# mosure/bevy_gaussian_splatting

Measured on NVIDIA H100. Metric: rendered Msplats/sec @1080p, 6M-gaussian cloud, higher is better.
Workload: dtype f32 (f16-packed inputs)

## Files before the change

bevy_gaussian_splatting_b200/csrc/raster.cu:

```cuda
#include <cuda_fp16.h>

#include "common.cuh"

namespace bgs {

constexpr int RT_THREADS = 256;
constexpr int RT_CHUNK = 256;

__device__ __forceinline__ void mbar_init(uint32_t bar, uint32_t count) {
    asm volatile("mbarrier.init.shared::cta.b64 [%0], %1;" ::"r"(bar), "r"(count) : "memory");
}
__device__ __forceinline__ void mbar_expect_tx(uint32_t bar, uint32_t bytes) {
    asm volatile("mbarrier.arrive.expect_tx.shared::cta.b64 _, [%0], %1;" ::"r"(bar), "r"(bytes) : "memory");
}
__device__ __forceinline__ void tma_bulk_g2s(uint32_t dst, const void* src, uint32_t bytes, uint32_t bar) {
    asm volatile("cp.async.bulk.shared::cluster.global.mbarrier::complete_tx::bytes [%0], [%1], %2, [%3];"
                 ::"r"(dst), "l"(src), "r"(bytes), "r"(bar) : "memory");
}
__device__ __forceinline__ void mbar_wait(uint32_t bar, uint32_t parity) {
    asm volatile(
        "{\n\t.reg .pred p;\n\t"
        "WAIT_%=:\n\t"
        "mbarrier.try_wait.parity.shared::cta.b64 p, [%0], %1;\n\t"
        "@p bra DONE_%=;\n\t"
        "bra WAIT_%=;\n\t"
        "DONE_%=:\n\t}" ::"r"(bar), "r"(parity) : "memory");
}
constexpr uint32_t ENT_WORDS = RT_CHUNK + 8;

struct PairStream {
    const uint32_t* entries;
    uint32_t (*ent)[ENT_WORDS];
    uint32_t a_ent, a_bar, end;
    bool tma;
    uint32_t issued = 0u, chunk = 0u;

    __device__ __forceinline__ PairStream(const uint32_t* tile_entries, uint32_t (*s_ent)[ENT_WORDS], unsigned long long* s_bar,
                                          uint2 range, bool use_tma)
        : entries(tile_entries), ent(s_ent), a_ent((uint32_t)__cvta_generic_to_shared(s_ent)),
          a_bar((uint32_t)__cvta_generic_to_shared(s_bar)), end(range.y), tma(use_tma) {
        if (!tma) return;
        if (threadIdx.x == 0) {
            mbar_init(a_bar, 1u); mbar_init(a_bar + 8u, 1u);
            asm volatile("fence.mbarrier_init.release.cluster;" ::: "memory");
        }
        __syncthreads();
        if (threadIdx.x == 0) issue(range.x, (uint32_t)RT_CHUNK, 0);
        issued = 1u;
    }
    __device__ __forceinline__ void issue(uint32_t base, uint32_t cnt, int buf) const {
        const uint32_t lead = base & 3u;
        const uint32_t bytes = ((lead + cnt) * 4u + 15u) & ~15u;
        mbar_expect_tx(a_bar + 8u * buf, bytes);
        tma_bulk_g2s(a_ent + (uint32_t)buf * ENT_WORDS * 4u, entries + (base - lead), bytes, a_bar + 8u * buf);
    }
    __device__ __forceinline__ void next(uint32_t base) {
        const int buf = (int)(chunk & 1u);
        if (tma) {
            if (base + RT_CHUNK < end) {
                if (threadIdx.x == 0) issue(base + RT_CHUNK, min((uint32_t)RT_CHUNK, end - base - RT_CHUNK), buf ^ 1);
                ++issued;
            }
            mbar_wait(a_bar + 8u * buf, (chunk >> 1) & 1u);
        }
    }
    template <class Index>
    __device__ __forceinline__ uint32_t entry(uint32_t base, Index j) const {
        return tma ? ent[chunk & 1u][(base & 3u) + j] : __ldg(entries + base + j);
    }
    __device__ __forceinline__ void finish() const {
        if (threadIdx.x == 0 && issued > chunk) mbar_wait(a_bar + 8u * (chunk & 1u), (chunk >> 1) & 1u);
    }
};

__device__ __forceinline__ void centre_out_tile(int b, int tiles_x, int tiles_y, int& tile_x, int& tile_y) {
    const int k = b / tiles_x, mid = tiles_y / 2;
    tile_x = b - k * tiles_x;
    tile_y = (k & 1) ? mid - (k + 1) / 2 : mid + k / 2;
}

__device__ __forceinline__ float linear_to_srgb(float c) {
    c = fminf(fmaxf(c, 0.0f), 1.0f);
    return c <= 0.0031308f ? 12.92f * c : 1.055f * __powf(c, 1.0f / 2.4f) - 0.055f;
}

constexpr uint32_t OUT_PREMUL = 1u, OUT_OVER = 2u;
__device__ __forceinline__ float srgb_decode(float c) {
    return c <= 0.04045f ? c * (1.0f / 12.92f) : __powf((c + 0.055f) * (1.0f / 1.055f), 2.4f);
}
__device__ __forceinline__ float4 read_pixel(const void* out, uint32_t fmt, size_t pix) {
    if (fmt == BGS_FORMAT_RGBA32F) return reinterpret_cast<const float4*>(out)[pix];
    if (fmt == BGS_FORMAT_RGBA16F) {
        const uint2 v = reinterpret_cast<const uint2*>(out)[pix];
        const float2 lo = __half22float2(*reinterpret_cast<const __half2*>(&v.x)), hi = __half22float2(*reinterpret_cast<const __half2*>(&v.y));
        return make_float4(lo.x, lo.y, hi.x, hi.y);
    }
    const uint32_t v = reinterpret_cast<const uint32_t*>(out)[pix];
    return make_float4(srgb_decode((float)(v & 255u) * (1.0f / 255.0f)), srgb_decode((float)((v >> 8) & 255u) * (1.0f / 255.0f)),
                       srgb_decode((float)((v >> 16) & 255u) * (1.0f / 255.0f)), (float)(v >> 24) * (1.0f / 255.0f));
}
__device__ __forceinline__ uint2 pack_rgba16f(float r, float g, float b, float a) {
    const __half2 lo = __floats2half2_rn(r, g), hi = __floats2half2_rn(b, a);
    return make_uint2(*reinterpret_cast<const uint32_t*>(&lo), *reinterpret_cast<const uint32_t*>(&hi));
}
__device__ __forceinline__ uint32_t pack_srgb8(float r, float g, float b, float a, bool with_alpha) {
    const uint32_t r8 = (uint32_t)(linear_to_srgb(r) * 255.0f + 0.5f);
    const uint32_t g8 = (uint32_t)(linear_to_srgb(g) * 255.0f + 0.5f);
    const uint32_t b8 = (uint32_t)(linear_to_srgb(b) * 255.0f + 0.5f);
    const uint32_t a8 = with_alpha ? (uint32_t)(fminf(fmaxf(a, 0.0f), 1.0f) * 255.0f + 0.5f) : 255u;
    return r8 | (g8 << 8) | (b8 << 16) | (a8 << 24);
}
__device__ __forceinline__ void write_pixel(void* out, uint32_t format, size_t pix, float r, float g, float b, float T) {
    const uint32_t fmt = format & 0xFFu, mode = format >> 8;
    float a = 1.0f;
    if (mode & OUT_OVER) {
        const float4 d = read_pixel(out, fmt, pix);
        r = fmaf(T, d.x, r); g = fmaf(T, d.y, g); b = fmaf(T, d.z, b);
        a = fmaf(T, d.w, 1.0f - T);
    } else if (mode & OUT_PREMUL) {
        a = 1.0f - T;
    }
    if (fmt == BGS_FORMAT_RGBA32F) {
        reinterpret_cast<float4*>(out)[pix] = make_float4(r, g, b, a);
    } else if (fmt == BGS_FORMAT_RGBA16F) {
        reinterpret_cast<uint2*>(out)[pix] = pack_rgba16f(r, g, b, a);
    } else {
        reinterpret_cast<uint32_t*>(out)[pix] = pack_srgb8(r, g, b, a, mode != 0);
    }
}

constexpr uint32_t SM_Q0 = 0;
constexpr uint32_t SM_UV = SM_Q0 + RT_CHUNK * 16;
constexpr uint32_t SM_Q2 = SM_UV + RT_CHUNK * 16;
constexpr uint32_t SM_LIST = SM_Q2 + RT_CHUNK * 16;
constexpr uint32_t SM_EXTRA = SM_LIST + (RT_THREADS / 32) * RT_CHUNK * 2;
constexpr uint32_t SM_BYTES = SM_EXTRA;
constexpr uint32_t SM_BYTES_2D = SM_EXTRA + 4 * RT_CHUNK * 16;

constexpr uint32_t REC_UV = SM_UV - SM_Q0, REC_Q2 = SM_Q2 - SM_Q0;
static_assert(REC_UV == RT_CHUNK * 16 && REC_Q2 == 2 * RT_CHUNK * 16, "q0, uv, q2 are consecutive float4 [RT_CHUNK] arrays");

__device__ __forceinline__ float4 lds4(uint32_t a) {
    float4 r; asm volatile("ld.shared.v4.f32 {%0,%1,%2,%3}, [%4];" : "=f"(r.x), "=f"(r.y), "=f"(r.z), "=f"(r.w) : "r"(a)); return r;
}
__device__ __forceinline__ float2 lds2(uint32_t a) {
    float2 r; asm volatile("ld.shared.v2.f32 {%0,%1}, [%2];" : "=f"(r.x), "=f"(r.y) : "r"(a)); return r;
}
__device__ __forceinline__ uint32_t lds_u16(uint32_t a) { uint32_t r; asm volatile("ld.shared.u16 %0, [%1];" : "=r"(r) : "r"(a)); return r; }
__device__ __forceinline__ uint32_t lds_u32(uint32_t a) { uint32_t r; asm volatile("ld.shared.u32 %0, [%1];" : "=r"(r) : "r"(a)); return r; }

__device__ __forceinline__ float2 quad_uv(float fx, float fy, float4 q0, float2 q1) {
    const float dx = __fsub_rn(fx, q0.x), dy = __fsub_rn(fy, q0.y);
    return make_float2(__fmaf_rn(q0.w, dy, __fmul_rn(q0.z, dx)), __fmaf_rn(q1.y, dy, __fmul_rn(q1.x, dx)));
}

template <class Hit>
__device__ __forceinline__ uint32_t compact_candidates(uint32_t cnt, unsigned short* list, uint32_t rec0, Hit hit) {
    uint32_t nl = 0;
    for (uint32_t j0 = 0; j0 < cnt; j0 += 32) {
        const uint32_t j = j0 + (threadIdx.x & 31u);
        bool h = false;
        if (j < cnt) h = hit(j);
        const uint32_t m = __ballot_sync(0xffffffffu, h);
        if (h) list[nl + __popc(m & lanemask_lt())] = (unsigned short)(rec0 + j * 16u);
        nl += __popc(m);
    }
    __syncwarp();
    return nl;
}

template <int MODE, bool AUX>
__global__ void __launch_bounds__(RT_THREADS, (MODE == 0 && !AUX) ? 6 : 5)
raster_kernel(const SplatRec* __restrict__ recs, const float4* __restrict__ extra, const uint32_t* __restrict__ tile_entries,
              const uint2* __restrict__ ranges, int W, int H, int tiles_x, void* __restrict__ out, uint32_t format,
              const float4* __restrict__ aux, void* __restrict__ out_depth, void* __restrict__ out_normal) {
    __shared__ __align__(16) unsigned char s_mem[(MODE == 2 ? SM_BYTES_2D : SM_BYTES) + (AUX ? 2 * RT_CHUNK * 16 : 0)];
    constexpr uint32_t SM_AUX = MODE == 2 ? SM_BYTES_2D : SM_BYTES;
    __shared__ __align__(16) uint32_t s_ent[2][ENT_WORDS];
    __shared__ __align__(8) unsigned long long s_bar[2];
    __shared__ __align__(8) float2 s_thr[MODE == 0 ? RT_CHUNK : 1];
    float4* s_q0 = reinterpret_cast<float4*>(s_mem + SM_Q0);
    float4* s_uv = reinterpret_cast<float4*>(s_mem + SM_UV);
    float4* s_q2 = reinterpret_cast<float4*>(s_mem + SM_Q2);
    const int t = threadIdx.x, lane = t & 31, warp = t >> 5;
    unsigned short* s_list = reinterpret_cast<unsigned short*>(s_mem + SM_LIST) + warp * RT_CHUNK;
    const uint32_t a_base = (uint32_t)__cvta_generic_to_shared(s_mem);
    const uint32_t a_list = a_base + SM_LIST + (uint32_t)warp * RT_CHUNK * 2u;
    int tile_x, tile_y;
    centre_out_tile((int)blockIdx.x, tiles_x, (int)gridDim.x / tiles_x, tile_x, tile_y);
    const int tile = tile_y * tiles_x + tile_x;
    const int wx0 = tile_x * TILE_PX + (warp & 1) * 8, wy0 = tile_y * TILE_PX + (warp >> 1) * 4;
    const int px = wx0 + (lane & 7), py = wy0 + (lane >> 3);
    const bool inside = px < W && py < H;
    const float fx = (float)px + 0.5f, fy = (float)py + 0.5f;
    const float rcx = (float)wx0 + 4.0f, rcy = (float)wy0 + 2.0f;
    const float tcx = (float)(tile_x * TILE_PX) + 8.0f, tcy = (float)(tile_y * TILE_PX) + 8.0f;
    uint2 range = ranges[tile];
    range.x = ~range.x;

    if (range.x >= range.y) {
        if (inside && !((format >> 8) & OUT_OVER)) {
            write_pixel(out, format, (size_t)py * W + px, 0.f, 0.f, 0.f, 1.0f);
            if (AUX) {
                write_pixel(out_depth, format, (size_t)py * W + px, 0.f, 0.f, 0.f, 1.0f);
                write_pixel(out_normal, format, (size_t)py * W + px, 0.f, 0.f, 0.f, 1.0f);
            }
        }
        return;
    }
    PairStream ps(tile_entries, s_ent, s_bar, range, range.y - range.x > (uint32_t)RT_CHUNK);

    float T = inside ? 1.0f : 0.0f, cr = 0.0f, cg = 0.0f, cb = 0.0f;
    float dr = 0.0f, dg = 0.0f, db = 0.0f, nr = 0.0f, ng = 0.0f, nb = 0.0f;
    for (uint32_t base = range.x; base < range.y; base += RT_CHUNK, ++ps.chunk) {
        if (__syncthreads_count(T < T_STOP ? 0 : 1) == 0) break;
        const uint32_t cnt = min((uint32_t)RT_CHUNK, range.y - base);
        ps.next(base);
        if ((uint32_t)t < cnt) {
            const uint32_t r = ps.entry(base, t);
            const float4* rp = reinterpret_cast<const float4*>(recs + r);
            const float4 p0 = __ldg(rp), p1 = __ldg(rp + 1);
            s_q0[t] = p0;
            s_uv[t] = p1;
            s_q2[t] = __ldg(rp + 2);
            if (MODE == 0) {
                const float ax = fabsf(p0.x - tcx) + 4.0f, ay = fabsf(p0.y - tcy) + 6.0f;
                const float ur = fabsf(p0.z) * 3.5f + fabsf(p0.w) * 1.5f, vr = fabsf(p1.x) * 3.5f + fabsf(p1.y) * 1.5f;
                const float um = fabsf(p0.z) * ax + fabsf(p0.w) * ay + ur, vm = fabsf(p1.x) * ax + fabsf(p1.y) * ay + vr;
                s_thr[t] = make_float2(ur + 1.0f + 1e-5f * um, vr + 1.0f + 1e-5f * vm);
            }
            if (MODE == 2) {
                float4* s_ex = reinterpret_cast<float4*>(s_mem + SM_EXTRA);
                const float4* ep = extra + (size_t)r * 4;
#pragma unroll
                for (int q = 0; q < 4; ++q) s_ex[q * RT_CHUNK + t] = __ldg(ep + q);
            }
            if (AUX) {
                float4* s_ax = reinterpret_cast<float4*>(s_mem + SM_AUX);
                s_ax[t] = __ldg(aux + (size_t)r * 2);
                s_ax[RT_CHUNK + t] = __ldg(aux + (size_t)r * 2 + 1);
            }
        }
        __syncthreads();
        const uint32_t nl = !__any_sync(0xffffffffu, !(T < T_STOP)) ? 0u : compact_candidates(cnt, s_list, a_base, [&](uint32_t j) {
            const float4 q = s_uv[j];
            const uint32_t bx = __float_as_uint(q.z), by = __float_as_uint(q.w);
            bool hit = !((int)(bx >> 16) < wx0 | (int)(bx & 0xFFFFu) > wx0 + 7 | (int)(by >> 16) < wy0 |
                         (int)(by & 0xFFFFu) > wy0 + 3);
            if (MODE == 0 && hit) {
                const float4 p = s_q0[j];
                const float2 th = s_thr[j];
                const float dxc = rcx - p.x, dyc = rcy - p.y;
                hit = !(fabsf(p.z * dxc + p.w * dyc) > th.x || fabsf(q.x * dxc + q.y * dyc) > th.y);
            }
            return hit;
        });
        if (MODE == 0 && !AUX) {
            const uint32_t a_end = a_list + nl * 2u;
            uint32_t a_it = a_list;
            float lim = (T < T_STOP) ? -1.0f : 1.0f;
            auto blend_if_covered = [&](uint32_t a_rec, float2 uv) {
                asm volatile(
                    "{\n\t"
                    ".reg .pred p, q;\n\t"
                    ".reg .f32 au, av, x, y, z, o, qd, e, a, w, na;\n\t"
                    "abs.f32 au, %5;\n\t"
                    "abs.f32 av, %6;\n\t"
                    "setp.le.f32 p, au, %4;\n\t"
                    "setp.le.and.f32 p, av, %4, p;\n\t"
                    "ld.shared.v4.f32 {x, y, z, o}, [%7+%8];\n\t"
                    "mul.rn.f32 qd, %5, %5;\n\t"
                    "fma.rn.f32 qd, %6, %6, qd;\n\t"
                    "mul.rn.f32 qd, qd, 0fC0CFBF83;\n\t"
                    "ex2.approx.ftz.f32 e, qd;\n\t"
                    "mul.rn.f32 a, e, o;\n\t"
                    "min.f32 a, a, 0f3F7FBE77;\n\t"
                    "mul.rn.f32 w, a, %0;\n\t"
                    "neg.f32 na, a;\n\t"
                    "@p fma.rn.f32 %1, w, x, %1;\n\t"
                    "@p fma.rn.f32 %2, w, y, %2;\n\t"
                    "@p fma.rn.f32 %3, w, z, %3;\n\t"
                    "@p fma.rn.f32 %0, na, %0, %0;\n\t"
                    "setp.lt.and.f32 q, %0, 0f38D1B717, p;\n\t"
                    "@q mov.f32 %4, 0fBF800000;\n\t"
                    "}"
                    : "+f"(T), "+f"(cr), "+f"(cg), "+f"(cb), "+f"(lim)
                    : "f"(uv.x), "f"(uv.y), "r"(a_rec), "n"(REC_Q2));
            };
            for (; a_it + 2u < a_end; a_it += 4u) {
                const uint32_t two = lds_u32(a_it);
                const uint32_t ra = two & 0xFFFFu, rb = two >> 16;
                const float4 pa = lds4(ra), pb = lds4(rb);
                const float2 sa = lds2(ra + REC_UV), sb = lds2(rb + REC_UV);
                const float2 uva = quad_uv(fx, fy, pa, sa), uvb = quad_uv(fx, fy, pb, sb);
                blend_if_covered(ra, uva);
                blend_if_covered(rb, uvb);
            }
            if (a_it != a_end) {
                const uint32_t ra = lds_u16(a_it);
                const float4 pa = lds4(ra);
                const float2 sa = lds2(ra + REC_UV);
                blend_if_covered(ra, quad_uv(fx, fy, pa, sa));
            }
        } else if (!(T < T_STOP)) {
            const uint32_t a_end = a_list + nl * 2u;
            for (uint32_t a_it = a_list; a_it != a_end; a_it += 2u) {
                const uint32_t a_rec = lds_u16(a_it);
                const float4 q0 = lds4(a_rec);
                const float2 q1 = lds2(a_rec + REC_UV);
                float e;
                float4 q2;
                if (MODE == 0) {
                    const float2 uv = quad_uv(fx, fy, q0, q1);
                    if (!(fabsf(uv.x) <= 1.0f && fabsf(uv.y) <= 1.0f)) continue;
                    const float qd = __fmaf_rn(uv.y, uv.y, __fmul_rn(uv.x, uv.x));
                    q2 = lds4(a_rec + REC_Q2);
                    asm("ex2.approx.ftz.f32 %0, %1;" : "=f"(e) : "f"(qd * -6.492127684f));
                } else {
                    const float dx = __fsub_rn(fx, q0.x), dy = __fsub_rn(fy, q0.y);
                    const float mx = __fadd_rn(dx, dx), my = -__fadd_rn(dy, dy);
                    const float Rq = q1.y;
                    float power;
                    if (MODE == 1) {
                        if (!(fabsf(mx) <= Rq && fabsf(my) <= Rq)) continue;
                        const float ddx = -mx, ddy = -my;
                        const float t1 = __fmul_rn(__fmul_rn(q0.z, ddx), ddx), t2 = __fmul_rn(__fmul_rn(q1.x, ddy), ddy);
                        power = __fadd_rn(__fmul_rn(-0.5f, __fadd_rn(t1, t2)), __fmul_rn(__fmul_rn(q0.w, ddx), ddy));
                    } else {
                        const float4 e0 = lds4(a_rec + SM_EXTRA);
                        if (!(fabsf(mx) <= e0.x && fabsf(my) <= e0.x)) continue;
                        const float4 e1 = lds4(a_rec + SM_EXTRA + RT_CHUNK * 16);
                        const float4 e2 = lds4(a_rec + SM_EXTRA + 2 * RT_CHUNK * 16);
                        const float4 e3 = lds4(a_rec + SM_EXTRA + 3 * RT_CHUNK * 16);
                        const float pcx = __fadd_rn(mx, e0.y), pcy = __fadd_rn(__fmul_rn(my, e0.w), e0.z);
                        const float hux = __fsub_rn(__fmul_rn(pcx, e3.x), e1.x), huy = __fsub_rn(__fmul_rn(pcx, e3.y), e1.y),
                                    huz = __fsub_rn(__fmul_rn(pcx, e3.z), e1.z);
                        const float hvx = __fsub_rn(__fmul_rn(pcy, e3.x), e2.x), hvy = __fsub_rn(__fmul_rn(pcy, e3.y), e2.y),
                                    hvz = __fsub_rn(__fmul_rn(pcy, e3.z), e2.z);
                        const float cpx = __fsub_rn(__fmul_rn(huy, hvz), __fmul_rn(huz, hvy));
                        const float cpy = __fsub_rn(__fmul_rn(huz, hvx), __fmul_rn(hux, hvz));
                        const float cpz = __fsub_rn(__fmul_rn(hux, hvy), __fmul_rn(huy, hvx));
                        const float us = __fdiv_rn(cpx, cpz), vs = __fdiv_rn(cpy, cpz);
                        const float s3 = __fadd_rn(__fmul_rn(us, us), __fmul_rn(vs, vs));
                        const float ex = __fsub_rn(e0.y, pcx), ey = __fsub_rn(e0.z, pcy);
                        const float s2 = __fmul_rn(2.0f, __fadd_rn(__fmul_rn(ex, ex), __fmul_rn(ey, ey)));
                        power = -__fmul_rn(0.5f, fminf(s3, s2));
                    }
                    if (power > 0.0f) continue;
                    q2 = lds4(a_rec + REC_Q2);
                    e = __expf(power);
                }
                const float a = fminf(e * q2.w, 0.999f);
                const float w = a * T;
                cr = fmaf(w, q2.x, cr); cg = fmaf(w, q2.y, cg); cb = fmaf(w, q2.z, cb);
                if (AUX) {
                    const float4 ad = lds4(a_rec + SM_AUX), an = lds4(a_rec + SM_AUX + RT_CHUNK * 16);
                    dr = fmaf(w, ad.x, dr); dg = fmaf(w, ad.y, dg); db = fmaf(w, ad.z, db);
                    nr = fmaf(w, an.x, nr); ng = fmaf(w, an.y, ng); nb = fmaf(w, an.z, nb);
                }
                T = fmaf(-a, T, T);
                if (T < T_STOP) break;
            }
        }
    }
    ps.finish();
    if (!inside) return;
    write_pixel(out, format, (size_t)py * W + px, cr, cg, cb, T);
    if (AUX) {
        write_pixel(out_depth, format, (size_t)py * W + px, dr, dg, db, T);
        write_pixel(out_normal, format, (size_t)py * W + px, nr, ng, nb, T);
    }
}

constexpr int R2_THREADS = 128;
constexpr uint32_t R2_LIST = SM_Q2 + RT_CHUNK * 16;
constexpr uint32_t R2_BYTES = R2_LIST + (R2_THREADS / 32) * RT_CHUNK * 2;

__device__ __forceinline__ void store_pixel2(void* out, uint32_t format, size_t pix, bool in0, bool in1, float r0, float g0,
                                             float b0, float r1, float g1, float b1, float T0, float T1) {
    if (format >> 8) {
        if (in0) write_pixel(out, format, pix, r0, g0, b0, T0);
        if (in1) write_pixel(out, format, pix + 1, r1, g1, b1, T1);
        return;
    }
    if (format == BGS_FORMAT_RGBA32F) {
        float4* o = reinterpret_cast<float4*>(out) + pix;
        if (in0) o[0] = make_float4(r0, g0, b0, 1.0f);
        if (in1) o[1] = make_float4(r1, g1, b1, 1.0f);
    } else if (format == BGS_FORMAT_RGBA16F) {
        uint2* o = reinterpret_cast<uint2*>(out) + pix;
        const uint2 p0 = pack_rgba16f(r0, g0, b0, 1.0f), p1 = pack_rgba16f(r1, g1, b1, 1.0f);
        if (in0) o[0] = p0;
        if (in1) o[1] = p1;
    } else {
        uint32_t* o = reinterpret_cast<uint32_t*>(out) + pix;
        const uint32_t p0 = pack_srgb8(r0, g0, b0, 1.0f, false), p1 = pack_srgb8(r1, g1, b1, 1.0f, false);
        if (in0 && in1 && (pix & 1) == 0) *reinterpret_cast<uint2*>(o) = make_uint2(p0, p1);
        else { if (in0) o[0] = p0; if (in1) o[1] = p1; }
    }
}

template <bool CHUNKED>
__global__ void __launch_bounds__(R2_THREADS)
raster2_kernel(const SplatRec* __restrict__ recs, const uint32_t* __restrict__ tile_entries, const uint2* __restrict__ ranges,
               int W, int H, int tiles_x, void* __restrict__ out, uint32_t format, float4* __restrict__ state,
               unsigned char* __restrict__ tile_done, uint32_t* __restrict__ tiles_done, int first, int last) {
    __shared__ __align__(16) unsigned char s_mem[R2_BYTES];
    float4* s_q0 = reinterpret_cast<float4*>(s_mem + SM_Q0);
    float4* s_uv = reinterpret_cast<float4*>(s_mem + SM_UV);
    float4* s_q2 = reinterpret_cast<float4*>(s_mem + SM_Q2);
    const int t = threadIdx.x, lane = t & 31, warp = t >> 5;
    unsigned short* s_list = reinterpret_cast<unsigned short*>(s_mem + R2_LIST) + warp * RT_CHUNK;
    const uint32_t a_base = (uint32_t)__cvta_generic_to_shared(s_mem);
    const uint32_t a_list = a_base + R2_LIST + (uint32_t)warp * RT_CHUNK * 2u;
    int tile_x, tile_y;
    centre_out_tile((int)blockIdx.x, tiles_x, (int)gridDim.x / tiles_x, tile_x, tile_y);
    const int tile = tile_y * tiles_x + tile_x;
    const int wy0 = tile_y * TILE_PX + warp * 4;
    const int px0 = tile_x * TILE_PX + 2 * (lane & 7), py = wy0 + (lane >> 3);
    const bool in0 = px0 < W && py < H, in1 = px0 + 1 < W && py < H;
    const float fx0 = (float)px0 + 0.5f, fx1 = (float)px0 + 1.5f, fy = (float)py + 0.5f;
    uint2 range = ranges[tile];
    range.x = ~range.x;

    float T0 = in0 ? 1.0f : 0.0f, T1 = in1 ? 1.0f : 0.0f;
    float lim0 = in0 ? 1.0f : -1.0f, lim1 = in1 ? 1.0f : -1.0f;
    float r0 = 0.f, g0 = 0.f, b0 = 0.f, r1 = 0.f, g1 = 0.f, b1 = 0.f;
    float4* st = nullptr;
    if (CHUNKED) {
        st = state + ((size_t)tile * R2_THREADS + t) * 2;
        if (!first) {
            const bool done = tile_done[tile] != 0;
            if (!last && (done || range.x >= range.y)) return;
            const float4 s0 = st[0], s1 = st[1];
            r0 = s0.x; g0 = s0.y; b0 = s0.z; T0 = s0.w;
            r1 = s1.x; g1 = s1.y; b1 = s1.z; T1 = s1.w;
            lim0 = (in0 && !(T0 < T_STOP)) ? 1.0f : -1.0f;
            lim1 = (in1 && !(T1 < T_STOP)) ? 1.0f : -1.0f;
            if (done) range.y = range.x;
        }
    }
    __shared__ __align__(16) uint32_t s_ent[2][ENT_WORDS];
    __shared__ __align__(8) unsigned long long s_bar[2];
    PairStream ps(tile_entries, s_ent, s_bar, range, range.y > range.x && range.y - range.x > (uint32_t)RT_CHUNK);
    for (uint32_t base = range.x; base < range.y; base += RT_CHUNK, ++ps.chunk) {
        if (__syncthreads_count((lim0 > 0.f || lim1 > 0.f) ? 1 : 0) == 0) break;
        const uint32_t cnt = min((uint32_t)RT_CHUNK, range.y - base);
        ps.next(base);
#pragma unroll
        for (int k = 0; k < RT_CHUNK / R2_THREADS; ++k) {
            const uint32_t j = t + k * R2_THREADS;
            if (j < cnt) {
                const uint32_t r = ps.entry(base, j);
                const float4* rp = reinterpret_cast<const float4*>(recs + r);
                s_q0[j] = __ldg(rp);
                s_uv[j] = __ldg(rp + 1);
                s_q2[j] = __ldg(rp + 2);
            }
        }
        __syncthreads();
        const uint32_t nl = !__any_sync(0xffffffffu, lim0 > 0.f || lim1 > 0.f) ? 0u : compact_candidates(cnt, s_list, 0u, [&](uint32_t j) {
            const uint32_t by = __float_as_uint(s_uv[j].w);
            return !((int)(by >> 16) < wy0 || (int)(by & 0xFFFFu) > wy0 + 3);
        });
        if (lim0 > 0.f || lim1 > 0.f) {
            const uint32_t a_end = a_list + nl * 2u;
            for (uint32_t a_it = a_list; a_it != a_end; a_it += 2u) {
                const uint32_t a_rec = a_base + lds_u16(a_it);
                const float4 q0 = lds4(a_rec);
                const float2 q1 = lds2(a_rec + REC_UV);
                const float2 uva = quad_uv(fx0, fy, q0, q1), uvb = quad_uv(fx1, fy, q0, q1);
                const bool ca = fabsf(uva.x) <= lim0 && fabsf(uva.y) <= lim0;
                const bool cb = fabsf(uvb.x) <= lim1 && fabsf(uvb.y) <= lim1;
                if (!(ca || cb)) continue;
                const float4 q2 = lds4(a_rec + REC_Q2);
                if (ca) {
                    float e;
                    asm("ex2.approx.ftz.f32 %0, %1;" : "=f"(e) : "f"(__fmaf_rn(uva.y, uva.y, __fmul_rn(uva.x, uva.x)) * -6.492127684f));
                    const float a = fminf(e * q2.w, 0.999f);
                    const float w = a * T0;
                    r0 = fmaf(w, q2.x, r0); g0 = fmaf(w, q2.y, g0); b0 = fmaf(w, q2.z, b0);
                    T0 = fmaf(-a, T0, T0);
                    if (T0 < T_STOP) lim0 = -1.0f;
                }
                if (cb) {
                    float e;
                    asm("ex2.approx.ftz.f32 %0, %1;" : "=f"(e) : "f"(__fmaf_rn(uvb.y, uvb.y, __fmul_rn(uvb.x, uvb.x)) * -6.492127684f));
                    const float a = fminf(e * q2.w, 0.999f);
                    const float w = a * T1;
                    r1 = fmaf(w, q2.x, r1); g1 = fmaf(w, q2.y, g1); b1 = fmaf(w, q2.z, b1);
                    T1 = fmaf(-a, T1, T1);
                    if (T1 < T_STOP) lim1 = -1.0f;
                }
                if (!(lim0 > 0.f || lim1 > 0.f)) break;
            }
        }
    }
    ps.finish();
    if (CHUNKED && !last) {
        st[0] = make_float4(r0, g0, b0, T0);
        st[1] = make_float4(r1, g1, b1, T1);
        if (__syncthreads_count((lim0 > 0.f || lim1 > 0.f) ? 1 : 0) == 0 && t == 0) {
            tile_done[tile] = 1;
            atomicAdd(tiles_done, 1u);
        }
        return;
    }
    if (!(in0 || in1)) return;
    store_pixel2(out, format, (size_t)py * W + px0, in0, in1, r0, g0, b0, r1, g1, b1, T0, T1);
}

void launch_raster(int mode, bool large_footprints, const SplatRec* recs, const float4* extra, const uint32_t* tile_entries,
                   const uint2* ranges, int W, int H, int tiles_x, int tiles_y, void* out, uint32_t format,
                   const float4* aux, void* out_depth, void* out_normal, cudaStream_t stream) {
    const int grid = tiles_x * tiles_y;
    if (aux == nullptr && mode == 0 && large_footprints) {
        raster2_kernel<false><<<grid, R2_THREADS, 0, stream>>>(recs, tile_entries, ranges, W, H, tiles_x, out, format,
                                                               nullptr, nullptr, nullptr, 1, 1);
        return;
    }
    static void (*const kernels[2][3])(const SplatRec*, const float4*, const uint32_t*, const uint2*, int, int, int, void*,
                                       uint32_t, const float4*, void*, void*) = {
        {raster_kernel<0, false>, raster_kernel<1, false>, raster_kernel<2, false>},
        {raster_kernel<0, true>, raster_kernel<1, true>, raster_kernel<2, true>}};
    kernels[aux != nullptr][mode == 0 ? 0 : mode == 1 ? 1 : 2]<<<grid, RT_THREADS, 0, stream>>>(
        recs, extra, tile_entries, ranges, W, H, tiles_x, out, format, aux, out_depth, out_normal);
}

void launch_raster_round(const SplatRec* recs, const uint32_t* tile_entries, const uint2* ranges, int W, int H, int tiles_x,
                         int tiles_y, void* out, uint32_t format, float4* state, unsigned char* tile_done,
                         uint32_t* tiles_done, int first, int last, cudaStream_t stream) {
    raster2_kernel<true><<<tiles_x * tiles_y, R2_THREADS, 0, stream>>>(recs, tile_entries, ranges, W, H, tiles_x, out, format,
                                                                       state, tile_done, tiles_done, first, last);
}

}
```

Baseline: 16470.

## Compute per-warp hit bitmasks at load time and gather candidates from shared masks

New measurement: 16790 (median of 6 runs). 1.02x the previous value.

```diff
diff --git a/bevy_gaussian_splatting_b200/csrc/raster.cu b/bevy_gaussian_splatting_b200/csrc/raster.cu
--- a/bevy_gaussian_splatting_b200/csrc/raster.cu
+++ b/bevy_gaussian_splatting_b200/csrc/raster.cu
@@ -154,17 +154,30 @@
     return make_float2(__fmaf_rn(q0.w, dy, __fmul_rn(q0.z, dx)), __fmaf_rn(q1.y, dy, __fmul_rn(q1.x, dx)));
 }
 
-template <class Hit>
-__device__ __forceinline__ uint32_t compact_candidates(uint32_t cnt, unsigned short* list, uint32_t rec0, Hit hit) {
-    uint32_t nl = 0;
-    for (uint32_t j0 = 0; j0 < cnt; j0 += 32) {
-        const uint32_t j = j0 + (threadIdx.x & 31u);
-        bool h = false;
-        if (j < cnt) h = hit(j);
-        const uint32_t m = __ballot_sync(0xffffffffu, h);
-        if (h) list[nl + __popc(m & lanemask_lt())] = (unsigned short)(rec0 + j * 16u);
-        nl += __popc(m);
-    }
+__device__ __forceinline__ void put_mask(unsigned char* s_mask, uint32_t j, uint32_t m) {
+    s_mask[(j & 31u) * 8u + (j >> 5)] = (unsigned char)m;
+}
+
+__device__ __forceinline__ uint32_t gather_candidates(const unsigned char* s_mask, uint32_t cnt, uint32_t rect, uint32_t a_list,
+                                                      uint32_t rec0) {
+    const uint32_t lane = threadIdx.x & 31u, lt = lanemask_lt();
+    const uint2 mw = reinterpret_cast<const uint2*>(s_mask)[lane];
+    const uint32_t lo = mw.x >> rect, hi = mw.y >> rect, e0 = rec0 + lane * 16u;
+    uint32_t a_end = a_list;
+#pragma unroll
+    for (uint32_t g = 0; g < RT_CHUNK / 32; ++g) {
+        if (g * 32u >= cnt) break;
+        const uint32_t w = g < 4u ? lo : hi, bit = 1u << (8u * (g & 3u));
+        uint32_t m;
+        asm volatile("{\n\t.reg .pred p;\n\t.reg .b32 k;\n\t"
+                     "and.b32 k, %1, %2;\n\tsetp.ne.u32 p, k, 0;\n\t"
+                     "vote.sync.ballot.b32 %0, p, 0xffffffff;\n\t"
+                     "and.b32 k, %0, %3;\n\tpopc.b32 k, k;\n\tmad.lo.u32 k, k, 2, %4;\n\t"
+                     "@p st.shared.u16 [k], %5;\n\t}"
+                     : "=r"(m) : "r"(w), "r"(bit), "r"(lt), "r"(a_end), "r"(e0 + g * 32u * 16u) : "memory");
+        a_end += __popc(m) * 2u;
+    }
+    const uint32_t nl = (a_end - a_list) >> 1;
     __syncwarp();
     return nl;
 }
@@ -178,22 +191,20 @@
     constexpr uint32_t SM_AUX = MODE == 2 ? SM_BYTES_2D : SM_BYTES;
     __shared__ __align__(16) uint32_t s_ent[2][ENT_WORDS];
     __shared__ __align__(8) unsigned long long s_bar[2];
-    __shared__ __align__(8) float2 s_thr[MODE == 0 ? RT_CHUNK : 1];
+    __shared__ __align__(8) unsigned char s_mask[RT_CHUNK];
     float4* s_q0 = reinterpret_cast<float4*>(s_mem + SM_Q0);
     float4* s_uv = reinterpret_cast<float4*>(s_mem + SM_UV);
     float4* s_q2 = reinterpret_cast<float4*>(s_mem + SM_Q2);
     const int t = threadIdx.x, lane = t & 31, warp = t >> 5;
-    unsigned short* s_list = reinterpret_cast<unsigned short*>(s_mem + SM_LIST) + warp * RT_CHUNK;
     const uint32_t a_base = (uint32_t)__cvta_generic_to_shared(s_mem);
     const uint32_t a_list = a_base + SM_LIST + (uint32_t)warp * RT_CHUNK * 2u;
     int tile_x, tile_y;
     centre_out_tile((int)blockIdx.x, tiles_x, (int)gridDim.x / tiles_x, tile_x, tile_y);
     const int tile = tile_y * tiles_x + tile_x;
-    const int wx0 = tile_x * TILE_PX + (warp & 1) * 8, wy0 = tile_y * TILE_PX + (warp >> 1) * 4;
-    const int px = wx0 + (lane & 7), py = wy0 + (lane >> 3);
+    const int tx0 = tile_x * TILE_PX, ty0 = tile_y * TILE_PX;
+    const int px = tx0 + (warp & 1) * 8 + (lane & 7), py = ty0 + (warp >> 1) * 4 + (lane >> 3);
     const bool inside = px < W && py < H;
     const float fx = (float)px + 0.5f, fy = (float)py + 0.5f;
-    const float rcx = (float)wx0 + 4.0f, rcy = (float)wy0 + 2.0f;
     const float tcx = (float)(tile_x * TILE_PX) + 8.0f, tcy = (float)(tile_y * TILE_PX) + 8.0f;
     uint2 range = ranges[tile];
     range.x = ~range.x;
@@ -216,6 +227,7 @@
         if (__syncthreads_count(T < T_STOP ? 0 : 1) == 0) break;
         const uint32_t cnt = min((uint32_t)RT_CHUNK, range.y - base);
         ps.next(base);
+        uint32_t mask = 0u;
         if ((uint32_t)t < cnt) {
             const uint32_t r = ps.entry(base, t);
             const float4* rp = reinterpret_cast<const float4*>(recs + r);
@@ -223,11 +235,21 @@
             s_q0[t] = p0;
             s_uv[t] = p1;
             s_q2[t] = __ldg(rp + 2);
-            if (MODE == 0) {
-                const float ax = fabsf(p0.x - tcx) + 4.0f, ay = fabsf(p0.y - tcy) + 6.0f;
-                const float ur = fabsf(p0.z) * 3.5f + fabsf(p0.w) * 1.5f, vr = fabsf(p1.x) * 3.5f + fabsf(p1.y) * 1.5f;
-                const float um = fabsf(p0.z) * ax + fabsf(p0.w) * ay + ur, vm = fabsf(p1.x) * ax + fabsf(p1.y) * ay + vr;
-                s_thr[t] = make_float2(ur + 1.0f + 1e-5f * um, vr + 1.0f + 1e-5f * vm);
+            const float ax = fabsf(p0.x - tcx) + 4.0f, ay = fabsf(p0.y - tcy) + 6.0f;
+            const float ur = fabsf(p0.z) * 3.5f + fabsf(p0.w) * 1.5f, vr = fabsf(p1.x) * 3.5f + fabsf(p1.y) * 1.5f;
+            const float um = fabsf(p0.z) * ax + fabsf(p0.w) * ay + ur, vm = fabsf(p1.x) * ax + fabsf(p1.y) * ay + vr;
+            const float thu = ur + 1.0f + 1e-5f * um, thv = vr + 1.0f + 1e-5f * vm;
+            const uint32_t bx = __float_as_uint(p1.z), by = __float_as_uint(p1.w);
+#pragma unroll
+            for (int w = 0; w < RT_THREADS / 32; ++w) {
+                const int wx0 = tx0 + (w & 1) * 8, wy0 = ty0 + (w >> 1) * 4;
+                bool hit = !((int)(bx >> 16) < wx0 | (int)(bx & 0xFFFFu) > wx0 + 7 | (int)(by >> 16) < wy0 |
+                             (int)(by & 0xFFFFu) > wy0 + 3);
+                if (MODE == 0) {
+                    const float dxc = ((float)wx0 + 4.0f) - p0.x, dyc = ((float)wy0 + 2.0f) - p0.y;
+                    hit &= !(fabsf(p0.z * dxc + p0.w * dyc) > thu | fabsf(p1.x * dxc + p1.y * dyc) > thv);
+                }
+                mask |= (uint32_t)hit << w;
             }
             if (MODE == 2) {
                 float4* s_ex = reinterpret_cast<float4*>(s_mem + SM_EXTRA);
@@ -241,20 +263,9 @@
                 s_ax[RT_CHUNK + t] = __ldg(aux + (size_t)r * 2 + 1);
             }
         }
+        put_mask(s_mask, t, mask);
         __syncthreads();
-        const uint32_t nl = !__any_sync(0xffffffffu, !(T < T_STOP)) ? 0u : compact_candidates(cnt, s_list, a_base, [&](uint32_t j) {
-            const float4 q = s_uv[j];
-            const uint32_t bx = __float_as_uint(q.z), by = __float_as_uint(q.w);
-            bool hit = !((int)(bx >> 16) < wx0 | (int)(bx & 0xFFFFu) > wx0 + 7 | (int)(by >> 16) < wy0 |
-                         (int)(by & 0xFFFFu) > wy0 + 3);
-            if (MODE == 0 && hit) {
-                const float4 p = s_q0[j];
-                const float2 th = s_thr[j];
-                const float dxc = rcx - p.x, dyc = rcy - p.y;
-                hit = !(fabsf(p.z * dxc + p.w * dyc) > th.x || fabsf(q.x * dxc + q.y * dyc) > th.y);
-            }
-            return hit;
-        });
+        const uint32_t nl = !__any_sync(0xffffffffu, !(T < T_STOP)) ? 0u : gather_candidates(s_mask, cnt, warp, a_list, a_base);
         if (MODE == 0 && !AUX) {
             const uint32_t a_end = a_list + nl * 2u;
             uint32_t a_it = a_list;
@@ -410,7 +421,6 @@
     float4* s_uv = reinterpret_cast<float4*>(s_mem + SM_UV);
     float4* s_q2 = reinterpret_cast<float4*>(s_mem + SM_Q2);
     const int t = threadIdx.x, lane = t & 31, warp = t >> 5;
-    unsigned short* s_list = reinterpret_cast<unsigned short*>(s_mem + R2_LIST) + warp * RT_CHUNK;
     const uint32_t a_base = (uint32_t)__cvta_generic_to_shared(s_mem);
     const uint32_t a_list = a_base + R2_LIST + (uint32_t)warp * RT_CHUNK * 2u;
     int tile_x, tile_y;
@@ -442,6 +452,7 @@
     }
     __shared__ __align__(16) uint32_t s_ent[2][ENT_WORDS];
     __shared__ __align__(8) unsigned long long s_bar[2];
+    __shared__ __align__(8) unsigned char s_mask[RT_CHUNK];
     PairStream ps(tile_entries, s_ent, s_bar, range, range.y > range.x && range.y - range.x > (uint32_t)RT_CHUNK);
     for (uint32_t base = range.x; base < range.y; base += RT_CHUNK, ++ps.chunk) {
         if (__syncthreads_count((lim0 > 0.f || lim1 > 0.f) ? 1 : 0) == 0) break;
@@ -450,19 +461,25 @@
 #pragma unroll
         for (int k = 0; k < RT_CHUNK / R2_THREADS; ++k) {
             const uint32_t j = t + k * R2_THREADS;
+            uint32_t mask = 0u;
             if (j < cnt) {
                 const uint32_t r = ps.entry(base, j);
                 const float4* rp = reinterpret_cast<const float4*>(recs + r);
+                const float4 p1 = __ldg(rp + 1);
                 s_q0[j] = __ldg(rp);
-                s_uv[j] = __ldg(rp + 1);
+                s_uv[j] = p1;
                 s_q2[j] = __ldg(rp + 2);
-            }
+                const uint32_t by = __float_as_uint(p1.w);
+#pragma unroll
+                for (int w = 0; w < R2_THREADS / 32; ++w) {
+                    const int wy0w = tile_y * TILE_PX + w * 4;
+                    mask |= (uint32_t)!((int)(by >> 16) < wy0w || (int)(by & 0xFFFFu) > wy0w + 3) << w;
+                }
+            }
+            put_mask(s_mask, j, mask);
         }
         __syncthreads();
-        const uint32_t nl = !__any_sync(0xffffffffu, lim0 > 0.f || lim1 > 0.f) ? 0u : compact_candidates(cnt, s_list, 0u, [&](uint32_t j) {
-            const uint32_t by = __float_as_uint(s_uv[j].w);
-            return !((int)(by >> 16) < wy0 || (int)(by & 0xFFFFu) > wy0 + 3);
-        });
+        const uint32_t nl = !__any_sync(0xffffffffu, lim0 > 0.f || lim1 > 0.f) ? 0u : gather_candidates(s_mask, cnt, warp, a_list, 0u);
         if (lim0 > 0.f || lim1 > 0.f) {
             const uint32_t a_end = a_list + nl * 2u;
             for (uint32_t a_it = a_list; a_it != a_end; a_it += 2u) {
```

## Split each warp into two 4x4 half-footprints with separate candidate lists

Applied to the files above, without the earlier changes.

After: 16540 before, 16670 after (median of 6 runs). No clear change (+0.8%).

```diff
diff --git a/bevy_gaussian_splatting_b200/csrc/raster.cu b/bevy_gaussian_splatting_b200/csrc/raster.cu
--- a/bevy_gaussian_splatting_b200/csrc/raster.cu
+++ b/bevy_gaussian_splatting_b200/csrc/raster.cu
@@ -136,6 +136,7 @@
 constexpr uint32_t SM_EXTRA = SM_LIST + (RT_THREADS / 32) * RT_CHUNK * 2;
 constexpr uint32_t SM_BYTES = SM_EXTRA;
 constexpr uint32_t SM_BYTES_2D = SM_EXTRA + 4 * RT_CHUNK * 16;
+constexpr uint32_t SM_BYTES_HALVES = SM_LIST + 2 * (RT_THREADS / 32) * RT_CHUNK * 2;
 
 constexpr uint32_t REC_UV = SM_UV - SM_Q0, REC_Q2 = SM_Q2 - SM_Q0;
 static_assert(REC_UV == RT_CHUNK * 16 && REC_Q2 == 2 * RT_CHUNK * 16, "q0, uv, q2 are consecutive float4 [RT_CHUNK] arrays");
@@ -169,12 +170,37 @@
     return nl;
 }
 
+template <class Hit>
+__device__ __forceinline__ uint2 compact_candidates2(uint32_t cnt, unsigned short* list0, unsigned short* list1, uint32_t rec0,
+                                                     Hit hit) {
+    uint32_t n0 = 0, n1 = 0;
+    for (uint32_t j0 = 0; j0 < cnt; j0 += 32) {
+        const uint32_t j = j0 + (threadIdx.x & 31u);
+        uint32_t h = 0;
+        if (j < cnt) h = hit(j);
+        const uint32_t m0 = __ballot_sync(0xffffffffu, h & 1u), m1 = __ballot_sync(0xffffffffu, h & 2u);
+        if (h & 1u) list0[n0 + __popc(m0 & lanemask_lt())] = (unsigned short)(rec0 + j * 16u);
+        if (h & 2u) list1[n1 + __popc(m1 & lanemask_lt())] = (unsigned short)(rec0 + j * 16u);
+        n0 += __popc(m0);
+        n1 += __popc(m1);
+    }
+    __syncwarp();
+    return make_uint2(n0, n1);
+}
+
+__device__ __forceinline__ bool sat_hit(float4 p, float vx, float vy, float2 th, float rcx, float rcy) {
+    const float dxc = rcx - p.x, dyc = rcy - p.y;
+    return !(fabsf(p.z * dxc + p.w * dyc) > th.x || fabsf(vx * dxc + vy * dyc) > th.y);
+}
+
 template <int MODE, bool AUX>
 __global__ void __launch_bounds__(RT_THREADS, (MODE == 0 && !AUX) ? 6 : 5)
 raster_kernel(const SplatRec* __restrict__ recs, const float4* __restrict__ extra, const uint32_t* __restrict__ tile_entries,
               const uint2* __restrict__ ranges, int W, int H, int tiles_x, void* __restrict__ out, uint32_t format,
               const float4* __restrict__ aux, void* __restrict__ out_depth, void* __restrict__ out_normal) {
-    __shared__ __align__(16) unsigned char s_mem[(MODE == 2 ? SM_BYTES_2D : SM_BYTES) + (AUX ? 2 * RT_CHUNK * 16 : 0)];
+    constexpr bool HALVES = MODE == 0 && !AUX;
+    __shared__ __align__(16) unsigned char s_mem[(MODE == 2 ? SM_BYTES_2D : HALVES ? SM_BYTES_HALVES : SM_BYTES) +
+                                                 (AUX ? 2 * RT_CHUNK * 16 : 0)];
     constexpr uint32_t SM_AUX = MODE == 2 ? SM_BYTES_2D : SM_BYTES;
     __shared__ __align__(16) uint32_t s_ent[2][ENT_WORDS];
     __shared__ __align__(8) unsigned long long s_bar[2];
@@ -183,14 +209,15 @@
     float4* s_uv = reinterpret_cast<float4*>(s_mem + SM_UV);
     float4* s_q2 = reinterpret_cast<float4*>(s_mem + SM_Q2);
     const int t = threadIdx.x, lane = t & 31, warp = t >> 5;
-    unsigned short* s_list = reinterpret_cast<unsigned short*>(s_mem + SM_LIST) + warp * RT_CHUNK;
+    const int half = HALVES ? lane >> 4 : 0;
+    unsigned short* s_list = reinterpret_cast<unsigned short*>(s_mem + SM_LIST) + (HALVES ? 2 * warp : warp) * RT_CHUNK;
     const uint32_t a_base = (uint32_t)__cvta_generic_to_shared(s_mem);
-    const uint32_t a_list = a_base + SM_LIST + (uint32_t)warp * RT_CHUNK * 2u;
+    const uint32_t a_list = a_base + SM_LIST + (uint32_t)((HALVES ? 2 * warp + half : warp) * RT_CHUNK * 2);
     int tile_x, tile_y;
     centre_out_tile((int)blockIdx.x, tiles_x, (int)gridDim.x / tiles_x, tile_x, tile_y);
     const int tile = tile_y * tiles_x + tile_x;
     const int wx0 = tile_x * TILE_PX + (warp & 1) * 8, wy0 = tile_y * TILE_PX + (warp >> 1) * 4;
-    const int px = wx0 + (lane & 7), py = wy0 + (lane >> 3);
+    const int px = HALVES ? wx0 + half * 4 + (lane & 3) : wx0 + (lane & 7), py = HALVES ? wy0 + ((lane >> 2) & 3) : wy0 + (lane >> 3);
     const bool inside = px < W && py < H;
     const float fx = (float)px + 0.5f, fy = (float)py + 0.5f;
     const float rcx = (float)wx0 + 4.0f, rcy = (float)wy0 + 2.0f;
@@ -209,6 +236,12 @@
         return;
     }
     PairStream ps(tile_entries, s_ent, s_bar, range, range.y - range.x > (uint32_t)RT_CHUNK);
+    if (HALVES) {
+        static_assert(SM_BYTES_HALVES - SM_LIST == RT_THREADS * 32, "two 16 B stores per thread fill the lists");
+        const uint4 z = make_uint4(a_base * 0x10001u, a_base * 0x10001u, a_base * 0x10001u, a_base * 0x10001u);
+        reinterpret_cast<uint4*>(s_mem + SM_LIST)[2 * t] = z;
+        reinterpret_cast<uint4*>(s_mem + SM_LIST)[2 * t + 1] = z;
+    }
 
     float T = inside ? 1.0f : 0.0f, cr = 0.0f, cg = 0.0f, cb = 0.0f;
     float dr = 0.0f, dg = 0.0f, db = 0.0f, nr = 0.0f, ng = 0.0f, nb = 0.0f;
@@ -224,8 +257,9 @@
             s_uv[t] = p1;
             s_q2[t] = __ldg(rp + 2);
             if (MODE == 0) {
-                const float ax = fabsf(p0.x - tcx) + 4.0f, ay = fabsf(p0.y - tcy) + 6.0f;
-                const float ur = fabsf(p0.z) * 3.5f + fabsf(p0.w) * 1.5f, vr = fabsf(p1.x) * 3.5f + fabsf(p1.y) * 1.5f;
+                constexpr float EX = HALVES ? 1.5f : 3.5f, OX = HALVES ? 6.0f : 4.0f;
+                const float ax = fabsf(p0.x - tcx) + OX, ay = fabsf(p0.y - tcy) + 6.0f;
+                const float ur = fabsf(p0.z) * EX + fabsf(p0.w) * 1.5f, vr = fabsf(p1.x) * EX + fabsf(p1.y) * 1.5f;
                 const float um = fabsf(p0.z) * ax + fabsf(p0.w) * ay + ur, vm = fabsf(p1.x) * ax + fabsf(p1.y) * ay + vr;
                 s_thr[t] = make_float2(ur + 1.0f + 1e-5f * um, vr + 1.0f + 1e-5f * vm);
             }
@@ -242,21 +276,40 @@
             }
         }
         __syncthreads();
-        const uint32_t nl = !__any_sync(0xffffffffu, !(T < T_STOP)) ? 0u : compact_candidates(cnt, s_list, a_base, [&](uint32_t j) {
-            const float4 q = s_uv[j];
-            const uint32_t bx = __float_as_uint(q.z), by = __float_as_uint(q.w);
-            bool hit = !((int)(bx >> 16) < wx0 | (int)(bx & 0xFFFFu) > wx0 + 7 | (int)(by >> 16) < wy0 |
-                         (int)(by & 0xFFFFu) > wy0 + 3);
-            if (MODE == 0 && hit) {
-                const float4 p = s_q0[j];
-                const float2 th = s_thr[j];
-                const float dxc = rcx - p.x, dyc = rcy - p.y;
-                hit = !(fabsf(p.z * dxc + p.w * dyc) > th.x || fabsf(q.x * dxc + q.y * dyc) > th.y);
-            }
-            return hit;
-        });
-        if (MODE == 0 && !AUX) {
-            const uint32_t a_end = a_list + nl * 2u;
+        const bool live = __any_sync(0xffffffffu, !(T < T_STOP));
+        uint2 nh = make_uint2(0u, 0u);
+        uint32_t nl = 0u;
+        if (HALVES) {
+            const int hx1 = wx0 + 4;
+            if (live) nh = compact_candidates2(cnt, s_list, s_list + RT_CHUNK, a_base, [&](uint32_t j) {
+                const float4 q = s_uv[j];
+                const uint32_t bx = __float_as_uint(q.z), by = __float_as_uint(q.w);
+                const int xlo = (int)(bx & 0xFFFFu), xhi = (int)(bx >> 16);
+                const bool yhit = !((int)(by >> 16) < wy0 | (int)(by & 0xFFFFu) > wy0 + 3);
+                bool h0 = yhit & !(xhi < wx0 | xlo > wx0 + 3), h1 = yhit & !(xhi < hx1 | xlo > hx1 + 3);
+                if (h0 | h1) {
+                    const float4 p = s_q0[j];
+                    const float2 th = s_thr[j];
+                    h0 = h0 && sat_hit(p, q.x, q.y, th, rcx - 2.0f, rcy);
+                    h1 = h1 && sat_hit(p, q.x, q.y, th, rcx + 2.0f, rcy);
+                }
+                return (uint32_t)h0 | (uint32_t)h1 << 1;
+            });
+        } else {
+            if (live) nl = compact_candidates(cnt, s_list, a_base, [&](uint32_t j) {
+                const float4 q = s_uv[j];
+                const uint32_t bx = __float_as_uint(q.z), by = __float_as_uint(q.w);
+                bool hit = !((int)(bx >> 16) < wx0 | (int)(bx & 0xFFFFu) > wx0 + 7 | (int)(by >> 16) < wy0 |
+                             (int)(by & 0xFFFFu) > wy0 + 3);
+                if (MODE == 0 && hit) {
+                    hit = sat_hit(s_q0[j], q.x, q.y, s_thr[j], rcx, rcy);
+                }
+                return hit;
+            });
+        }
+        if (HALVES) {
+            const uint32_t n_me = half ? nh.y : nh.x, n_min = min(nh.x, nh.y), n_max = max(nh.x, nh.y);
+            const uint32_t a_both = a_list + (n_min & ~1u) * 2u, a_end = a_list + n_max * 2u, a_mine = a_list + n_me * 2u;
             uint32_t a_it = a_list;
             float lim = (T < T_STOP) ? -1.0f : 1.0f;
             auto blend_if_covered = [&](uint32_t a_rec, float2 uv) {
@@ -287,21 +340,19 @@
                     : "+f"(T), "+f"(cr), "+f"(cg), "+f"(cb), "+f"(lim)
                     : "f"(uv.x), "f"(uv.y), "r"(a_rec), "n"(REC_Q2));
             };
-            for (; a_it + 2u < a_end; a_it += 4u) {
+            auto blend_two = [&](uint32_t a_it, bool ends) {
                 const uint32_t two = lds_u32(a_it);
                 const uint32_t ra = two & 0xFFFFu, rb = two >> 16;
                 const float4 pa = lds4(ra), pb = lds4(rb);
                 const float2 sa = lds2(ra + REC_UV), sb = lds2(rb + REC_UV);
                 const float2 uva = quad_uv(fx, fy, pa, sa), uvb = quad_uv(fx, fy, pb, sb);
+                if (ends && a_it >= a_mine) lim = -1.0f;
                 blend_if_covered(ra, uva);
+                if (ends && a_it + 2u >= a_mine) lim = -1.0f;
                 blend_if_covered(rb, uvb);
-            }
-            if (a_it != a_end) {
-                const uint32_t ra = lds_u16(a_it);
-                const float4 pa = lds4(ra);
-                const float2 sa = lds2(ra + REC_UV);
-                blend_if_covered(ra, quad_uv(fx, fy, pa, sa));
-            }
+            };
+            for (; a_it != a_both; a_it += 4u) blend_two(a_it, false);
+            for (; a_it < a_end; a_it += 4u) blend_two(a_it, true);
         } else if (!(T < T_STOP)) {
             const uint32_t a_end = a_list + nl * 2u;
             for (uint32_t a_it = a_list; a_it != a_end; a_it += 2u) {
```
